# csm-kr/faster_rcnn_pytorch

Hardware: AMD Instinct MI355X
Metric: train images/sec (VGG16 Faster R-CNN, 600x1000, bs=1/GPU) (higher is better)
Workload: dtype f32; 1 GPU; VGG16 Faster R-CNN train step, synthetic 600x1000 frames, bs=1/GPU, HIP proposal/RoI path (N=20646 anchors, pre/post NMS 12000/2000, 128 RoIs, RoIPool 7x7 on 512x37x62); global_batch=1, parallelism=dp1, submission=eager (one launch per kernel), sampling=device-philox

## Files before the change

### faster_rcnn_pytorch_amd/csrc/rpn_conv_f32.hip

```cpp
#include "frcnn_common.h"
#include "frcnn_internal.h"
#include "frcnn_layout.h"
#include <algorithm>
#include <atomic>
#include <cstdlib>
#include <cstring>
#include <type_traits>
FRCNN_LAYOUT_STAMP(rpn_conv_f32);

typedef float f32x16 __attribute__((ext_vector_type(16)));

#define CF_MT 128
#define CF_NT 128
#define CF_CI 4
#define CF_KK (CF_CI * 9)
#define CF_AS 37
#define CF_RS 144
#define CF_ROWS (CF_CI * 3)
#define CF_SLAB (CF_MT * CF_NT)
#define CF_MAX_TILES 32768

struct CfLevel { const float *x; float *y; int H, W, HW, tile0; };
struct CfArgs {
    CfLevel lv[FRCNN_MAX_LEVELS];
    int n_levels, C, n_co_tiles, n_pos_tiles, Kc, n_units, G, pos_major;
};
struct CfTile { const float *x; float *y; int W, HW, p0, co0, tile; };

__device__ __forceinline__ CfTile cf_tile(const CfArgs &a, int t)
{
    int ct, pt;
    if (a.pos_major) { pt = t / a.n_co_tiles; ct = t - pt * a.n_co_tiles; }
    else { ct = t / a.n_pos_tiles; pt = t - ct * a.n_pos_tiles; }
    int l = 0;
#pragma unroll
    for (int q = 1; q < FRCNN_MAX_LEVELS; ++q) l += (q < a.n_levels && pt >= a.lv[q].tile0) ? 1 : 0;
    CfTile T;
    T.x = a.lv[l].x; T.y = a.lv[l].y; T.W = a.lv[l].W; T.HW = a.lv[l].HW;
    T.p0 = (pt - a.lv[l].tile0) * CF_NT;
    T.co0 = ct * CF_MT;
    T.tile = t;
    return T;
}

__device__ __forceinline__ long long cf_start(int s, int U, int G) { return ((long long)s * U) / G; }

#ifndef CF_WPS
#define CF_WPS 2
#endif
__global__ __launch_bounds__(256, CF_WPS) void rpn_conv3x3_f32_kernel(CfArgs a, const float *__restrict__ w, float *__restrict__ part, int *__restrict__ cnt)
{
    __shared__ float sA[2][CF_MT * CF_AS];
    __shared__ float sB[2][CF_ROWS * CF_RS];
    __shared__ int s_last;
    const int tid = threadIdx.x, lane = tid & 63, wave = __builtin_amdgcn_readfirstlane(tid >> 6);
    const int wm = wave >> 1, wn = wave & 1, li = lane & 31, lh = lane >> 5;
    const int G = a.G, U = a.n_units, Kc = a.Kc;
    const int sigma = (G % 8 == 0) ? (int)(blockIdx.x & 7) * (G >> 3) + (int)(blockIdx.x >> 3) : (int)blockIdx.x;
    const int u0 = (int)cf_start(sigma, U, G), u1 = (int)cf_start(sigma + 1, U, G);
    if (u0 >= u1) return;
    const int Ktot = a.C * 9;

    unsigned a_off[5];
    int a_lds[5];
#pragma unroll
    for (int q = 0; q < 5; ++q) {
        const int idx = tid + 256 * q, row = idx / 9, pc = idx - row * 9;
        a_off[q] = (unsigned)(row * Ktot + pc * 4);
        a_lds[q] = row * CF_AS + pc * 4;
    }
    const int hi = tid >> 7, bj = tid & 127;
    const int h_row = (tid >> 1) % CF_ROWS, h_ci = h_row / 3, h_dy = h_row - 3 * h_ci - 1, h_j = (tid & 1) ? CF_NT : -1;
    const bool a_tail = tid < 128, b_tail = tid < 2 * CF_ROWS;
    float4 ra[5];
    float rb[7];
    unsigned rb_ok = 0;
    auto issue_loads = [&](const CfTile &T, int chunk) {
        const float *wb = w + (size_t)T.co0 * Ktot + chunk * CF_KK;
        const float *xb = T.x + (size_t)chunk * CF_CI * T.HW;
#pragma unroll
        for (int q = 0; q < 5; ++q)
            if (q < 4 || a_tail) ra[q] = *(const float4 *)(wb + a_off[q]);
        unsigned okm = 0;
#pragma unroll
        for (int q = 0; q < 7; ++q) {
            int ci, dy, j;
            if (q < 6) { ci = hi ? (2 * q + 1) / 3 : (2 * q) / 3; dy = hi ? (2 * q + 1) % 3 - 1 : (2 * q) % 3 - 1; j = bj; }
            else { ci = h_ci; dy = h_dy; j = h_j; }
            const int f = T.p0 + j + dy * T.W;
            const bool ok = f >= 0 && f < T.HW && (q < 6 || b_tail);
// ... 480 lines not shown
#pragma unroll
                for (int i = 0; i < 3; ++i)
#pragma unroll
                    for (int j = 0; j < 3; ++j) w9[i][j] = wc[(i - 1) * (wt + 2) + (j - 1)];
#pragma unroll
                for (int r = 0; r < IN; ++r)
#pragma unroll
                    for (int q = 0; q < IN; ++q) {
                        const int tr = r == 0 ? 0 : (r <= M ? 1 : 2), br = r == 0 ? M - 1 : (r <= M ? r - 1 : 0);
                        const int tc = q == 0 ? 0 : (q <= M ? 1 : 2), bc = q == 0 ? M - 1 : (q <= M ? q - 1 : 0);
                        d[r][q] = ((w9[tr][tc] >> (br * M + bc)) & 1u) ? d[r][q] : 0.0f;
                    }
            }
        }
        if (MODE == 1) {
#pragma unroll
            for (int r = 0; r < IN; ++r)
#pragma unroll
                for (int q = 0; q < IN; ++q) bsum += d[r][q];
        }
        float wv[A][IN];
#pragma unroll
        for (int q = 0; q < IN; ++q) {
            float col[IN], o[A];
#pragma unroll
            for (int r = 0; r < IN; ++r) col[r] = d[r][q];
            if (MODE != 1) wn_bt<M>(col, o); else wn_a<M>(col, o);
#pragma unroll
            for (int r = 0; r < A; ++r) wv[r][q] = o[r];
        }
        const size_t at = col0 + (size_t)(ty0 + rr) * tw + tx0 + txl;
#pragma unroll
        for (int r = 0; r < A; ++r) {
            float o[A];
            if (MODE != 1) wn_bt<M>(wv[r], o); else wn_a<M>(wv[r], o);
#pragma unroll
#if defined(WN_TABL) && (WN_TABL & 2)
            for (int q = 0; q < A; ++q) if (o[q] == 1.2345e-30f) V[(size_t)(r * A + q) * plane + at] = o[q];
#else
            for (int q = 0; q < A; ++q) V[(size_t)(r * A + q) * plane + at] = o[q];
#endif
        }
        if (MODE == 2) {
            float w2[A][M];
#pragma unroll
            for (int r = 0; r < M; ++r)
#pragma unroll
                for (int q = 0; q < M; ++q) bsum += d[r + 1][q + 1];
#pragma unroll
            for (int q = 0; q < M; ++q) {
                float col[M], o[A];
#pragma unroll
                for (int r = 0; r < M; ++r) col[r] = d[r + 1][q + 1];
                wn_a<M>(col, o);
#pragma unroll
                for (int r = 0; r < A; ++r) w2[r][q] = o[r];
            }
#pragma unroll
            for (int r = 0; r < A; ++r) {
                float o[A];
                wn_a<M>(w2[r], o);
#pragma unroll
                for (int q = 0; q < A; ++q) a.out2[(size_t)(r * A + q) * plane + at] = o[q];
            }
        }
    }
    if (MODE != 0 && a.db_part) {
        __shared__ float red[4];
#pragma unroll
        for (int h = 32; h > 0; h >>= 1) bsum += __shfl_down(bsum, h, 64);
        if ((threadIdx.x & 63) == 0) red[threadIdx.x >> 6] = bsum;
        __syncthreads();
        if (threadIdx.x == 0) a.db_part[(size_t)c * st.first[FRCNN_MAX_LEVELS] + blockIdx.x] = (red[0] + red[1]) + (red[2] + red[3]);
    }
    if (a.zero_pad && strip == 0) {
        const int T = a.lv[l].T, Tp = (T + a.tg - 1) / a.tg * a.tg, np = Tp - T;
        for (int e = threadIdx.x; e < P * np; e += 256) {
            const int xi = e / np, q = e - xi * np;
            (MODE == 2 ? a.out2 : V)[(size_t)xi * plane + col0 + T + q] = 0.0f;
        }
    }
}

template <int M, bool POOL>
__device__ __forceinline__ void wn_output_tile(const WnArgs &a, int c, int t, const float (&mv)[Wn<M>::P])
{
    constexpr int A = Wn<M>::A;
    int l = 0;
#pragma unroll
    for (int q = 1; q < FRCNN_MAX_LEVELS; ++q) l += (q < a.n_levels && t >= a.lv[q].off) ? 1 : 0;
    const int tl = t - a.lv[l].off;
    if (tl >= a.lv[l].T) return;
    const size_t at = (size_t)c * a.Ttot + t;
    float s[M][A];
#pragma unroll
    for (int q = 0; q < A; ++q) {
        float col[A], o[M];
#pragma unroll
        for (int r = 0; r < A; ++r) col[r] = mv[r * A + q];
        wn_at<M>(col, o);
#pragma unroll
        for (int i = 0; i < M; ++i) s[i][q] = o[i];
    }
    const float b = a.bias ? a.bias[c] : 0.0f;
    const int H = a.lv[l].H, W = a.lv[l].W, ty = tl / a.lv[l].tw, tx = tl - ty * a.lv[l].tw;
    unsigned word = 0;
    if (POOL) {
        float v[M][M];
#pragma unroll
        for (int i = 0; i < M; ++i) {
            float o[M];
            wn_at<M>(s[i], o);
#pragma unroll
            for (int j = 0; j < M; ++j) { const float t = o[j] + b; v[i][j] = t < 0.0f ? 0.0f : t; }
        }
        const int Hp = H >> 1, Wp = W >> 1;
        float *yp = a.lv[l].y + (size_t)c * Hp * Wp;
#pragma unroll
        for (int wi = 0; wi < 2; ++wi)
#pragma unroll
            for (int wj = 0; wj < 2; ++wj) {
                const int py = 2 * ty + wi, px = 2 * tx + wj;
                if (py < Hp && px < Wp) {
                    float mx = v[2 * wi][2 * wj];
                    unsigned arg = 0;
                    if (v[2 * wi][2 * wj + 1] > mx || v[2 * wi][2 * wj + 1] != v[2 * wi][2 * wj + 1]) { mx = v[2 * wi][2 * wj + 1]; arg = 1; }
                    if (v[2 * wi + 1][2 * wj] > mx || v[2 * wi + 1][2 * wj] != v[2 * wi + 1][2 * wj]) { mx = v[2 * wi + 1][2 * wj]; arg = 2; }
                    if (v[2 * wi + 1][2 * wj + 1] > mx || v[2 * wi + 1][2 * wj + 1] != v[2 * wi + 1][2 * wj + 1]) { mx = v[2 * wi + 1][2 * wj + 1]; arg = 3; }
                    yp[(size_t)py * Wp + px] = mx;
                    word |= (arg | (mx > 0.0f ? 4u : 0u)) << (3 * (wi * 2 + wj));
                }
            }
        if (a.bits_out) a.bits_out[at] = (unsigned short)word;
        return;
    }
    float *y = a.lv[l].y + (size_t)c * H * W + (size_t)(M * ty) * W + M * tx;
    const bool vec = (W % M) == 0 && ((size_t)a.lv[l].y & (4 * M - 1)) == 0, pairs = (W & 1) == 0 && ((size_t)a.lv[l].y & 7) == 0;
#pragma unroll
    for (int i = 0; i < M; ++i) {
        float o[M];
        wn_at<M>(s[i], o);
        if (M * ty + i < H) {
            float v[M];
#pragma unroll
            for (int j = 0; j < M; ++j) {
                v[j] = o[j] + b;
                if (a.relu) v[j] = v[j] < 0.0f ? 0.0f : v[j];
                if (M * tx + j < W) word |= (v[j] > 0.0f) ? (1u << (i * M + j)) : 0u;
            }
            if (vec) {
                if (M == 4) *(float4 *)(y + (size_t)i * W) = make_float4(v[0], v[1], v[2], v[3]);
                else *(float2 *)(y + (size_t)i * W) = make_float2(v[0], v[1]);
            } else if (M == 4 && pairs) {
#pragma unroll
                for (int j = 0; j < M; j += 2)
                    if (M * tx + j < W) *(float2 *)(y + (size_t)i * W + j) = make_float2(v[j], v[j + 1]);
            } else {
#pragma unroll
                for (int j = 0; j < M; ++j)
                    if (M * tx + j < W) y[(size_t)i * W + j] = v[j];
            }
        }
    }
    if (a.bits_out) a.bits_out[at] = (unsigned short)word;
}

template <int M, bool POOL>
__global__ __launch_bounds__(256) void rpn_wino_output_kernel(WnArgs a, const float *__restrict__ Mp)
{
    static_assert(!POOL || M == 4, "fused pooling: 4 x 4 tiles only");
    constexpr int A = Wn<M>::A, P = Wn<M>::P;
    const int t = blockIdx.x * 256 + threadIdx.x, c = blockIdx.y;
    if (t >= a.Ttot) return;
    const size_t plane = (size_t)a.C * a.Ttot, at = (size_t)c * a.Ttot + t;
    float mv[P];
#pragma unroll
    for (int q = 0; q < A; ++q)
#pragma unroll
        for (int r = 0; r < A; ++r) {
#if defined(WN_TABL) && (WN_TABL & 4)
            mv[r * A + q] = (float)(r + q); asm volatile("" : "+v"(mv[r * A + q]));
#else
            mv[r * A + q] = Mp[(size_t)(r * A + q) * plane + at];
#endif
        }
    wn_output_tile<M, POOL>(a, c, t, mv);
}

template <int M>
__global__ __launch_bounds__(256) void rpn_wino_dw_kernel(const float *__restrict__ dU, float *__restrict__ dw, unsigned n, float *__restrict__ db,
                                                          const float *__restrict__ db_part, int n_strips)
{
    constexpr int A = Wn<M>::A;
    const unsigned dw_blocks = (n + 255u) / 256u;
    if (blockIdx.x >= dw_blocks) {
        __shared__ float red[256];
        const unsigned c = blockIdx.x - dw_blocks;
        float t = 0.0f;
        for (int i = threadIdx.x; i < n_strips; i += 256) t += db_part[(size_t)c * n_strips + i];
        red[threadIdx.x] = t;
        __syncthreads();
#pragma unroll
        for (int h = 128; h > 0; h >>= 1) {
            if ((int)threadIdx.x < h) red[threadIdx.x] += red[threadIdx.x + h];
            __syncthreads();
        }
        if (threadIdx.x == 0) db[c] = red[0];
        return;
    }
    const unsigned o = blockIdx.x * 256u + threadIdx.x;
    if (o >= n) return;
    float t[3][A];
#pragma unroll
    for (int q = 0; q < A; ++q) {
        float col[A], w3[3];
#pragma unroll
        for (int r = 0; r < A; ++r) col[r] = dU[(size_t)(r * A + q) * n + o];
        wn_gt<M>(col, w3);
#pragma unroll
        for (int i = 0; i < 3; ++i) t[i][q] = w3[i];
    }
#pragma unroll
    for (int i = 0; i < 3; ++i) {
        float w3[3];
        wn_gt<M>(t[i], w3);
#pragma unroll
        for (int j = 0; j < 3; ++j) dw[(size_t)o * 9 + i * 3 + j] = w3[j];
    }
}

#ifdef WN_STAMP
__device__ unsigned long long wn_stamps[4 * 1024];
extern "C" __attribute__((visibility("default"))) int frcnn_debug_wn_stamps(unsigned long long *out)
{
    return (int)hipMemcpyFromSymbol(out, HIP_SYMBOL(wn_stamps), sizeof(wn_stamps));
}
#define WN_STAMP_AT(i) do { if (threadIdx.x == 0) wn_stamps[blockIdx.x * 4 + (i)] = wall_clock64(); } while (0)
#else
#define WN_STAMP_AT(i) do { } while (0)
#endif
typedef short wn_bf16x8 __attribute__((ext_vector_type(8)));
typedef unsigned wn_u32x4 __attribute__((ext_vector_type(4)));
__device__ __forceinline__ void wn_cut8(const float *v, wn_u32x4 &h, wn_u32x4 &m, wn_u32x4 &l)
{
#pragma unroll
    for (int p = 0; p < 4; ++p) {
        const unsigned x0 = __builtin_bit_cast(unsigned, v[2 * p]), x1 = __builtin_bit_cast(unsigned, v[2 * p + 1]);
// ... 242 lines not shown
            const int fsw = (li >> 1) & 7;
            f32x4 fa[2][MI], fb[2][NI];
            auto fetch4 = [&](int j, int slot) {
                const int o = (((4 * lh + j) ^ fsw) << 2);
#pragma unroll
                for (int mi = 0; mi < MI; ++mi) fa[slot][mi] = *(const f32x4 *)(ra + mi * 32 * WN_KC + o);
#pragma unroll
                for (int ni = 0; ni < NI; ++ni) fb[slot][ni] = *(const f32x4 *)(rb + ni * 32 * WN_KC + o);
            };
            fetch4(0, 0);
#pragma unroll
            for (int j = 0; j < 4; ++j) {
                const int slot = j & 1;
                if (j + 1 < 4) fetch4(j + 1, slot ^ 1);
#pragma unroll
                for (int e = 0; e < 4; ++e) {
                    __builtin_amdgcn_sched_barrier(0);
#pragma unroll
                    for (int mi = 0; mi < MI; ++mi)
#pragma unroll
                        for (int ni = 0; ni < NI; ++ni)
                            acc[mi][ni] = __builtin_amdgcn_mfma_f32_32x32x2f32(fa[slot][mi][e], fb[slot][ni][e], acc[mi][ni], 0, 0, 0);
                    __builtin_amdgcn_sched_barrier(0);
                    WN_PIECE(4 * j + e);
                }
                __builtin_amdgcn_sched_barrier(0);
            }
        } else {
            const float *pa = &sA[buf][lh * MT + wm * (MT / 2) + MI * li];
            const float *pb = &sB[buf][lh * NW + wn * (NW / 2) + NI * li];
            float oa[2][MI], ob[2][NI];
            auto fetch = [&](int s, int slot) {
#if defined(WN_ABL) && (WN_ABL & 4)
#pragma unroll
                for (int mi = 0; mi < MI; ++mi) { oa[slot][mi] = (float)s; asm volatile("" : "+v"(oa[slot][mi])); }
#pragma unroll
                for (int ni = 0; ni < NI; ++ni) { ob[slot][ni] = (float)s; asm volatile("" : "+v"(ob[slot][ni])); }
                return;
#endif
                if constexpr (MI == 2) { const float2 t = *(const float2 *)(pa + 2 * s * MT); oa[slot][0] = t.x; oa[slot][1] = t.y; }
                else oa[slot][0] = pa[2 * s * MT];
                if constexpr (NI == 2) { const float2 t = *(const float2 *)(pb + 2 * s * NW); ob[slot][0] = t.x; ob[slot][1] = t.y; }
                else ob[slot][0] = pb[2 * s * NW];
            };
            fetch(0, 0);
#pragma unroll
            for (int s = 0; s < 16; ++s) {
                const int slot = s & 1;
                if (s + 1 < 16) fetch(s + 1, slot ^ 1);
                __builtin_amdgcn_sched_barrier(0);
#pragma unroll
                for (int mi = 0; mi < MI; ++mi)
#pragma unroll
                    for (int ni = 0; ni < NI; ++ni)
                        acc[mi][ni] = __builtin_amdgcn_mfma_f32_32x32x2f32(oa[slot][mi], ob[slot][ni], acc[mi][ni], 0, 0, 0);
                __builtin_amdgcn_sched_barrier(0);
                WN_PIECE(s);
            }
        }
#undef WN_PIECE
        if (!more || ntile != tile) {
            if (!more) WN_STAMP_AT(2);
            if constexpr (SPLIT) {
#pragma unroll
                for (int mi = 0; mi < MI; ++mi)
#pragma unroll
                    for (int ni = 0; ni < NI; ++ni) acc[mi][ni] += accs[mi][ni];
            }
            finish_segment(T, seg_first, chunk + 1 - seg_first);
            if (!more) WN_STAMP_AT(3);
            zero_acc();
            seg_first = 0;
            if (more) T = Tn;
        }
        tile = ntile; chunk = nchunk;
        asm volatile("s_waitcnt vmcnt(0)" ::: "memory");
#if !(defined(WN_ABL) && (WN_ABL & 8))
        __syncthreads();
#endif
    }
}

typedef float wn_f32x4 __attribute__((ext_vector_type(4)));
#define WO_TB 32
#define WO_NB 4
__device__ __forceinline__ void wn_dma16(const float *g, const float *lds)
{
    const unsigned l = (unsigned)(size_t)(const __attribute__((address_space(3))) float *)lds;
    asm volatile("s_mov_b32 m0, %0\n\ts_nop 0\n\tglobal_load_lds_dwordx4 %1, off" ::"s"(__builtin_amdgcn_readfirstlane(l)), "v"(g) : "memory");
}
template <int K, bool POOL>
__global__ __launch_bounds__(256, 1) void rpn_wino_gemm_out64_kernel(WnArgs a, const float *__restrict__ U, const float *__restrict__ V)
{
    constexpr int P = 36, MO = 64, NS = K / 4, bufF = K * (MO + WO_TB), NB = WO_NB;
    constexpr int TPW = K / 16 + K / 32;
    extern __shared__ __attribute__((aligned(16))) float wo_s[];
    const int tid = threadIdx.x, lane = tid & 63, wave = __builtin_amdgcn_readfirstlane(tid >> 6), i16 = lane & 15, kk = lane >> 4;
    const int t0 = blockIdx.x * WO_TB;
    const size_t sU = (size_t)K * MO, sV = (size_t)K * a.Ttot;
    auto issue = [&](int xi, int buf) {
        float *sA = wo_s + buf * bufF, *sB = sA + K * MO;
        const float *u = U + (size_t)xi * sU, *v = V + (size_t)xi * sV + t0;
#pragma unroll
        for (int q = 0; q < K / 16; ++q) {
            const int d = wave + 4 * q, r = lane >> 4, c = ((lane & 15) * 4 - 16 * r) & 63;
            wn_dma16(u + (size_t)(4 * d + r) * MO + c, sA + d * 256);
        }
#pragma unroll
        for (int q = 0; q < K / 32; ++q) {
            const int d = wave + 4 * q, r = lane >> 3, c = ((lane & 7) * 4 - 16 * ((r & 3) >> 1)) & 31;
            wn_dma16(v + (size_t)(8 * d + r) * a.Ttot + c, sB + d * 256);
        }
    };
    wn_f32x4 acc[P][2];
#pragma unroll
    for (int xi = 0; xi < P; ++xi) { acc[xi][0] = (wn_f32x4){0.0f, 0.0f, 0.0f, 0.0f}; acc[xi][1] = (wn_f32x4){0.0f, 0.0f, 0.0f, 0.0f}; }
#pragma unroll
    for (int xi = 0; xi < NB - 1; ++xi) issue(xi, xi);
#pragma unroll
    for (int xi = 0; xi < P; ++xi) {
        {
            const int fl = (P - 1 - xi) < (NB - 2) ? (P - 1 - xi) : (NB - 2);
            static_assert(NB - 2 <= 2, "counted waits below");
            if (fl == 2) asm volatile("s_waitcnt vmcnt(%0)" ::"n"(2 * TPW) : "memory");
            else if (fl == 1) asm volatile("s_waitcnt vmcnt(%0)" ::"n"(TPW) : "memory");
            else asm volatile("s_waitcnt vmcnt(0)" ::: "memory");
        }
        __syncthreads();
#if !(defined(WO_ABL) && (WO_ABL & 1))
        if (xi + NB - 1 < P) issue(xi + NB - 1, (xi + NB - 1) % NB);
#endif
        const float *sA = wo_s + (xi % NB) * bufF, *sB = sA + K * MO;
        const float *pa = sA + kk * MO + ((wave * 16 + i16 + 16 * kk) & 63);
        const float *pb0 = sB + kk * WO_TB + ((i16 + 16 * (kk >> 1)) & 31), *pb1 = sB + kk * WO_TB + ((16 + i16 + 16 * (kk >> 1)) & 31);
#pragma unroll
        for (int s = 0; s < NS; ++s) {
            const float av = pa[s * 4 * MO], b0 = pb0[s * 4 * WO_TB], b1 = pb1[s * 4 * WO_TB];
#if defined(WO_ABL) && (WO_ABL & 2)
            if (s > 0) continue;
#endif
            acc[xi][0] = __builtin_amdgcn_mfma_f32_16x16x4f32(av, b0, acc[xi][0], 0, 0, 0);
            acc[xi][1] = __builtin_amdgcn_mfma_f32_16x16x4f32(av, b1, acc[xi][1], 0, 0, 0);
        }
    }
#pragma unroll
    for (int tb = 0; tb < 2; ++tb)
#pragma unroll
        for (int r = 0; r < 4; ++r) {
            float mv[P];
#pragma unroll
            for (int xi = 0; xi < P; ++xi) mv[xi] = acc[xi][tb][r];
            wn_output_tile<4, POOL>(a, wave * 16 + 4 * kk + r, t0 + 16 * tb + i16, mv);
        }
}

static std::atomic<int> g_wn_products{[] { const char *e = getenv("FRCNN_CONV_F32_PRODUCTS"); return (e && (!strcmp(e, "split") || !strcmp(e, "1"))) ? 1 : 0; }()};
FRCNN_EXPORT int frcnn_conv3x3_f32_products(int mode)
{
    if (mode < 0) return g_wn_products.load();
    return g_wn_products.exchange(mode ? 1 : 0);
}

static int wn_launch_gemm(bool nt, int MT, int NW, const WgArgs &g, float *part, int *cnt, hipStream_t s)
{
    const bool split = g_wn_products.load() != 0;
#define WN_GEMM_CASE(NTv, MTv, NWv)                                                                                          \
    if (nt == NTv && MT == MTv && NW == NWv) {                                                                               \
        if (split) FRCNN_LAUNCH((rpn_wino_gemm_kernel<NTv, MTv, NWv, true>), dim3((unsigned)g.G), dim3(256), 0, s, g, part, cnt);   \
        else FRCNN_LAUNCH((rpn_wino_gemm_kernel<NTv, MTv, NWv, false>), dim3((unsigned)g.G), dim3(256), 0, s, g, part, cnt); \
        FRCNN_CHECK_LAUNCH("rpn_wino_gemm_kernel");                                                                          \
        return FRCNN_OK;                                                                                                     \
    }
    WN_GEMM_CASE(false, 128, 128)
    WN_GEMM_CASE(false, 64, 128)
    WN_GEMM_CASE(false, 128, 64)
    WN_GEMM_CASE(false, 64, 64)
    WN_GEMM_CASE(true, 128, 128)
    WN_GEMM_CASE(true, 128, 64)
    WN_GEMM_CASE(true, 64, 128)
    WN_GEMM_CASE(true, 64, 64)
#undef WN_GEMM_CASE
    return frcnn_set_error(FRCNN_ERR_UNSUPPORTED, "conv3x3_f32: no GEMM for a %d x %d tile", MT, NW);
}

#define CW_TC 16
#define CW_YS 17
#define CW_XS 19
#define CW_YB (32 * CW_YS)
#define CW_XB (32 * CW_XS)
#define CW_WAVE_LDS (2 * CW_YB + 4 * CW_XB)

struct CwLevel { const float *x; const float *dy; int H, W, HW, n_strips, unit0; };
struct CwArgs {
    CwLevel lv[FRCNN_MAX_LEVELS];
    int n_levels, C, n_units, S;
};

#ifndef CW_WPS
#define CW_WPS 1
#endif
__global__ __launch_bounds__(256, CW_WPS) void rpn_conv3x3_f32_wgrad_kernel(CwArgs a, float *__restrict__ dw, float *__restrict__ part, int *__restrict__ cnt)
{
    __shared__ float s_all[4 * CW_WAVE_LDS];
    __shared__ int s_last;
    const int tid = threadIdx.x, lane = tid & 63, wave = __builtin_amdgcn_readfirstlane(tid >> 6);
    const int li = lane & 31, lh = lane >> 5;
    const int C = a.C, nt = C / 32;
    const int tile = (int)blockIdx.x / a.S, split = (int)blockIdx.x - tile * a.S;
    const int co0 = (tile / nt) * 32, ci0 = (tile % nt) * 32;
    float *sY = s_all + wave * CW_WAVE_LDS, *sX = sY + 2 * CW_YB;
    const int q = split * 4 + wave, nq = a.S * 4;
    const int u0 = (int)(((long long)q * a.n_units) / nq), u1 = (int)(((long long)(q + 1) * a.n_units) / nq);

    f32x16 acc[9];
#pragma unroll
    for (int t = 0; t < 9; ++t)
#pragma unroll
        for (int r = 0; r < 16; ++r) acc[t][r] = 0.0f;

    const int sr = lane >> 1, sh = lane & 1;
    float *wy = sY + sr * CW_YS + sh * 8;
    float *wx = sX + sr * CW_XS + sh * 9;
    unsigned yo[8], xo[9];
    unsigned ymask = 0, xmask = 0;
    int lvl = 0, strip = 0, row = 0, H = 1, W = 1;
    const float *xg = nullptr, *yg = nullptr;
    auto decode = [&](int u) {
        int l = 0;
#pragma unroll
        for (int k = 1; k < FRCNN_MAX_LEVELS; ++k) l += (k < a.n_levels && u >= a.lv[k].unit0) ? 1 : 0;
        const int v = u - a.lv[l].unit0;
        lvl = l; H = a.lv[l].H; W = a.lv[l].W; xg = a.lv[l].x; yg = a.lv[l].dy;
        strip = v / H; row = v - strip * H;
        const int HW = a.lv[l].HW, c0 = strip * CW_TC;
        ymask = 0; xmask = 0;
#pragma unroll
// ... 257 lines not shown
}
FRCNN_EXPORT size_t frcnn_rpn_conv3x3_f32_workspace(const int *H_host, const int *W_host, int n_levels, int C)
{
    if (C <= 0 || C % CF_MT != 0) return 0;
    return frcnn_conv3x3_f32_workspace(H_host, W_host, n_levels, C, C);
}

template <int M>
static int wn_strips(WnStrips *st, const WnArgs &a, const int *H, int n_levels, long long channels, int halo, size_t *lds_bytes, int sm = M)
{
    int n_strips = 0;
    for (int per_block = Wn<M>::TPB; per_block >= 256; per_block /= 2) {
        n_strips = 0;
        for (int l = 0; l < FRCNN_MAX_LEVELS; ++l) {
            st->first[l] = n_strips;
            const int tw = l < n_levels ? a.lv[l].tw : 1, th = l < n_levels ? (H[l] + M - 1) / M : 1;
            st->segs[l] = (tw + Wn<M>::WT - 1) / Wn<M>::WT;
            st->rows[l] = std::min(128, std::max(1, per_block / std::min(tw, Wn<M>::WT)));
            if (l < n_levels) n_strips += st->segs[l] * ((th + st->rows[l] - 1) / st->rows[l]);
        }
        st->first[FRCNN_MAX_LEVELS] = n_strips;
        if ((long long)n_strips * channels >= 4096) break;
    }
    size_t fl = 0;
    for (int l = 0; l < n_levels; ++l) {
        const int wt = std::min(a.lv[l].tw, Wn<M>::WT), th = (H[l] + M - 1) / M, nr = std::min(st->rows[l], th);
        fl = std::max(fl, (size_t)(sm * nr + 2 * halo) * (size_t)(sm * wt + 2 * halo));
    }
    *lds_bytes = fl * sizeof(float);
    return n_strips;
}

template <int M>
static int wn_run(const float *const *in, float *const *out, const unsigned short *bits_in, const int *H, const int *W, int n_levels, int Cin, int Cout,
                  const float *w, bool transposed, const float *bias, int relu, unsigned short *bits_out, float *xt, void *workspace, hipStream_t s,
                  bool pooled = false, const float *u_rot = nullptr, float *dm_out = nullptr, bool want_bias = false)
{
    constexpr int P = Wn<M>::P;
    const int K = transposed ? Cout : Cin, Mo = transposed ? Cin : Cout;
    WnArgs a;
    const long long Ttot = wn_fill(&a, M, in, out, H, W, n_levels);
    a.bits = bits_in;
    FRCNN_REQUIRE(Ttot < (1ll << 24) && (long long)P * std::max(K, Mo) * Ttot < (1ll << 31) * 4, "conv3x3_f32: %lld output tiles are too many", Ttot);
    const CfWs ws = wn_carve(workspace, Cin, Cout, M, Ttot);
    const int MT = Mo % CF_MT == 0 ? CF_MT : 64;
    const int n_m_tiles = Mo / MT, n_t_tiles = (int)(Ttot / a.tg), Kc = K / WN_KC;
    const long long n_tiles = (long long)P * n_m_tiles * n_t_tiles, units = n_tiles * Kc;
    FRCNN_REQUIRE(n_tiles <= CF_MAX_TILES && units < (1ll << 31), "conv3x3_f32: %lld tiles above the limit %d", n_tiles, CF_MAX_TILES);
    const unsigned wb = (unsigned)((Mo / 16) * (K / 16));
    const float *Uuse = ws.U;
    if (transposed && u_rot) Uuse = u_rot;
    else {
        FRCNN_LAUNCH(rpn_wino_weight_kernel<M>, dim3(!transposed && u_rot ? 2 * wb : wb), dim3(256), 0, s, w, ws.U, (float *)u_rot, Cout, Cin, transposed ? 1 : 0);
        FRCNN_CHECK_LAUNCH("rpn_wino_weight_kernel");
    }
    a.C = K;
    float *Vb = xt ? xt : ws.V;
    a.zero_pad = xt ? 1 : 0;
    WnStrips st;
    size_t lds = 0;
    FRCNN_REQUIRE(!pooled || M == 4, "conv3x3_f32: a pooled gradient on the %d x %d tile", M, M);
    const int n_strips = wn_strips<M>(&st, a, H, n_levels, K, 1, &lds, pooled ? 2 : M);
    if (dm_out) {
        a.out2 = dm_out; a.zero_pad = 1;
        if (want_bias) {
            const size_t C9 = (size_t)((std::max(Cin, Cout) + CF_MT - 1) / CF_MT) * CF_MT;
            FRCNN_REQUIRE((size_t)K * n_strips <= C9 * C9 * 9, "conv3x3_f32_bwd_data: %d strips are too many for the bias partials", n_strips);
            a.db_part = ws.wt;
        }
        if (pooled) {
            if constexpr (M == 4) FRCNN_LAUNCH((rpn_wino_input_kernel<4, 2, true>), dim3((unsigned)n_strips, (unsigned)K), dim3(256), lds, s, a, st, Vb);
        } else FRCNN_LAUNCH((rpn_wino_input_kernel<M, 2, false>), dim3((unsigned)n_strips, (unsigned)K), dim3(256), lds, s, a, st, Vb);
    } else if (pooled) {
        if constexpr (M == 4) FRCNN_LAUNCH((rpn_wino_input_kernel<4, 0, true>), dim3((unsigned)n_strips, (unsigned)K), dim3(256), lds, s, a, st, Vb);
    } else FRCNN_LAUNCH((rpn_wino_input_kernel<M, 0, false>), dim3((unsigned)n_strips, (unsigned)K), dim3(256), lds, s, a, st, Vb);
    FRCNN_CHECK_LAUNCH("rpn_wino_input_kernel");
    if constexpr (M == 4) {
        static const bool no_fuse = [] { const char *e = getenv("FRCNN_WINO_NO_FUSE"); return e && atoi(e) != 0; }();
        if (Mo == 64 && K == 64 && !no_fuse) {
            a.C = Mo; a.bias = bias; a.relu = relu; a.bits_out = bits_out;
            const size_t wl = (size_t)WO_NB * K * (64 + WO_TB) * sizeof(float);
            if (relu == 2) (void)hipFuncSetAttribute((const void *)rpn_wino_gemm_out64_kernel<64, true>, hipFuncAttributeMaxDynamicSharedMemorySize, (int)wl);
            else (void)hipFuncSetAttribute((const void *)rpn_wino_gemm_out64_kernel<64, false>, hipFuncAttributeMaxDynamicSharedMemorySize, (int)wl);
            const dim3 gr((unsigned)(Ttot / WO_TB));
            if (relu == 2) FRCNN_LAUNCH((rpn_wino_gemm_out64_kernel<64, true>), gr, dim3(256), wl, s, a, Uuse, Vb);
            else FRCNN_LAUNCH((rpn_wino_gemm_out64_kernel<64, false>), gr, dim3(256), wl, s, a, Uuse, Vb);
            FRCNN_CHECK_LAUNCH("rpn_wino_gemm_out64_kernel");
            return FRCNN_OK;
        }
    }
    WgArgs g = {Uuse, Vb, ws.M, (long long)Mo * K, (long long)K * Ttot, (long long)Mo * Ttot, Mo, (int)Ttot, (int)Ttot,
                n_m_tiles, n_t_tiles, Kc, (int)units, (int)std::min<long long>(cf_ranges(), units), 0};
    {
        const long long per = (n_tiles + g.G - 1) / g.G;
        if (n_tiles >= 2ll * g.G && per * g.G * 100 <= n_tiles * 116) g.whole = 1;
        else if (n_tiles <= g.G && n_tiles * WN_ONE_TILE_DEN >= (long long)g.G * WN_ONE_TILE_NUM) { g.G = (int)n_tiles; g.whole = 1; }
    }
    { const int rc = wn_launch_gemm(false, MT, a.tg, g, ws.part, ws.cnt, s); if (rc) return rc; }
    a.C = Mo; a.bias = bias; a.relu = relu; a.bits_out = bits_out;
    if (relu == 2) {
        if constexpr (M == 4) FRCNN_LAUNCH((rpn_wino_output_kernel<4, true>), dim3((unsigned)((Ttot + 255) / 256), (unsigned)Mo), dim3(256), 0, s, a, ws.M);
    } else FRCNN_LAUNCH((rpn_wino_output_kernel<M, false>), dim3((unsigned)((Ttot + 255) / 256), (unsigned)Mo), dim3(256), 0, s, a, ws.M);
    FRCNN_CHECK_LAUNCH("rpn_wino_output_kernel");
    return FRCNN_OK;
}

static int cf_check(const void *const *p0, const void *const *p1, const int *H, const int *W, int n_levels, int Cin, int Cout, int in_mult, int out_mult,
                    const void *w, void *ws, size_t ws_bytes, const char *what)
{
    FRCNN_REQUIRE(p0 && p1 && H && W && w && ws, "%s: NULL pointer", what);
    FRCNN_REQUIRE(n_levels >= 1 && n_levels <= FRCNN_MAX_LEVELS, "%s: 1 <= n_levels <= %d", what, FRCNN_MAX_LEVELS);
    if (!wn_dims_ok(Cin, Cout) || Cin % in_mult != 0 || Cout % out_mult != 0)
        return frcnn_set_error(FRCNN_ERR_UNSUPPORTED, "%s: Cin=%d / Cout=%d must be multiples of %d / %d", what, Cin, Cout, in_mult, out_mult);
    for (int l = 0; l < n_levels; ++l) {
        FRCNN_REQUIRE(p0[l] && p1[l] && H[l] > 0 && W[l] > 0, "%s: bad level %d", what, l);
        FRCNN_REQUIRE((long long)H[l] * W[l] * std::max(Cin, Cout) < (1ll << 31), "%s: level %d too large", what, l);
    }
    const size_t need = frcnn_conv3x3_f32_workspace(H, W, n_levels, Cin, Cout);
    if (ws_bytes < need) return frcnn_set_error(FRCNN_ERR_WORKSPACE, "%s: workspace %zu < %zu bytes", what, ws_bytes, need);
    return FRCNN_OK;
}

FRCNN_EXPORT int frcnn_conv3x3_f32_fwd(const float *const *x_dev, float *const *y_dev, const int *H_host, const int *W_host, int n_levels, int Cin, int Cout,
                                       const float *w_dev, const float *bias_dev, int relu, unsigned short *relu_bits_dev, float *x_transformed_dev, float *u_rotated_dev,
                                       void *workspace, size_t workspace_bytes, void *stream)
{
    int rc = cf_check((const void *const *)x_dev, (const void *const *)y_dev, H_host, W_host, n_levels, Cin, Cout, WN_KC, 64, w_dev, workspace, workspace_bytes,
                      "conv3x3_f32_fwd");
    if (rc) return rc;
    FRCNN_REQUIRE(relu >= 0 && relu <= 2, "conv3x3_f32_fwd: relu = %d (0 none, 1 ReLU, 2 ReLU + max_pool2d(2, 2))", relu);
    if (relu == 2 && wn_pick_m(H_host, W_host, n_levels) != 4)
        return frcnn_set_error(FRCNN_ERR_UNSUPPORTED, "conv3x3_f32_fwd: the fused max-pool needs the 4 x 4 tile (frcnn_conv3x3_f32_tile_size)");
    if (wn_pick_m(H_host, W_host, n_levels) == 4)
        return wn_run<4>(x_dev, y_dev, nullptr, H_host, W_host, n_levels, Cin, Cout, w_dev, false, bias_dev, relu, relu_bits_dev, x_transformed_dev, workspace, (hipStream_t)stream,
                         false, u_rotated_dev);
    return wn_run<2>(x_dev, y_dev, nullptr, H_host, W_host, n_levels, Cin, Cout, w_dev, false, bias_dev, relu, relu_bits_dev, x_transformed_dev, workspace, (hipStream_t)stream,
                     false, u_rotated_dev);
}

FRCNN_EXPORT int frcnn_conv3x3_f32_supported(const int *H_host, const int *W_host, int n_levels, int Cin, int Cout, int need_grads)
{
    if (!H_host || !W_host || n_levels < 1 || n_levels > FRCNN_MAX_LEVELS || !wn_dims_ok(Cin, Cout) || Cout % 64 != 0 || (need_grads && Cin % 64 != 0)) return 0;
    const int M = wn_pick_m(H_host, W_host, n_levels), P = (M + 2) * (M + 2), Cm = std::max(Cin, Cout);
    WnArgs a;
    const long long Ttot = wn_fill(&a, M, nullptr, nullptr, H_host, W_host, n_levels);
    for (int l = 0; l < n_levels; ++l)
        if (H_host[l] <= 0 || W_host[l] <= 0 || (long long)H_host[l] * W_host[l] * Cm >= (1ll << 31)) return 0;
    if (Ttot >= (1ll << 24) || (long long)P * Cm * Ttot >= (1ll << 31) * 4) return 0;
    auto side = [](long long c) { return c % CF_MT == 0 ? c / CF_MT : c / 64; };
    auto tiles_ok = [&](long long mt, long long nt, long long k_chunks) {
        const long long n = P * mt * nt;
        return n <= CF_MAX_TILES && n * k_chunks < (1ll << 31);
    };
    if (!tiles_ok(side(Cout), Ttot / a.tg, Cin / WN_KC)) return 0;
    if (need_grads && (!tiles_ok(side(Cin), Ttot / a.tg, Cout / WN_KC) || !tiles_ok(side(Cout), side(Cin), Ttot / WN_KC))) return 0;
    return 1;
}

FRCNN_EXPORT int frcnn_conv3x3_f32_tile_size(const int *H_host, const int *W_host, int n_levels)
{
    if (!H_host || !W_host || n_levels < 1 || n_levels > FRCNN_MAX_LEVELS) return 0;
    return wn_pick_m(H_host, W_host, n_levels);
}

FRCNN_EXPORT size_t frcnn_conv3x3_f32_relu_bits_words(const int *H_host, const int *W_host, int n_levels, int Cout)
{
    if (!H_host || !W_host || n_levels < 1 || n_levels > FRCNN_MAX_LEVELS || Cout <= 0) return 0;
    WnArgs a;
    return (size_t)Cout * (size_t)wn_fill(&a, wn_pick_m(H_host, W_host, n_levels), nullptr, nullptr, H_host, W_host, n_levels);
// ... 172 lines not shown
```

Measured before the change: 154.0 images/s.

## Make fused Winograd GEMM+output kernel persistent with 512 threads and streaming inverse transform

Reworks the fused 64-channel Winograd GEMM/output kernel into a persistent kernel. Each block covers a contiguous range of 16-tile groups in passes of 64 tiles and uses 8 waves. The DMA ring carries on across passes, and addresses are passed as SGPR bases. Planes are consumed in column order so the inverse transform accumulates row by row, replacing 36 live accumulators per tile with 6 partial accumulators plus a 4x4 output. The aim is to cut register pressure, raise per-block tile width and overlap loads across passes; the cost is a more intricate counted-wait schedule and a grid sized to the CU count.

```diff
diff --git a/faster_rcnn_pytorch_amd/csrc/rpn_conv_f32.hip b/faster_rcnn_pytorch_amd/csrc/rpn_conv_f32.hip
--- a/faster_rcnn_pytorch_amd/csrc/rpn_conv_f32.hip
+++ b/faster_rcnn_pytorch_amd/csrc/rpn_conv_f32.hip
@@ -6,6 +6,7 @@
 #include <cstdlib>
 #include <cstring>
 #include <type_traits>
+#include <utility>
 FRCNN_LAYOUT_STAMP(rpn_conv_f32);
 
 typedef float f32x16 __attribute__((ext_vector_type(16)));
@@ -652,38 +653,26 @@
     }
 }
 
+__device__ __forceinline__ bool wn_tile_level(const WnArgs &a, int t, int &l, int &tl)
+{
+    l = 0;
+#pragma unroll
+    for (int q = 1; q < FRCNN_MAX_LEVELS; ++q) l += (q < a.n_levels && t >= a.lv[q].off) ? 1 : 0;
+    tl = t - a.lv[l].off;
+    return tl < a.lv[l].T;
+}
 template <int M, bool POOL>
-__device__ __forceinline__ void wn_output_tile(const WnArgs &a, int c, int t, const float (&mv)[Wn<M>::P])
-{
-    constexpr int A = Wn<M>::A;
-    int l = 0;
-#pragma unroll
-    for (int q = 1; q < FRCNN_MAX_LEVELS; ++q) l += (q < a.n_levels && t >= a.lv[q].off) ? 1 : 0;
-    const int tl = t - a.lv[l].off;
-    if (tl >= a.lv[l].T) return;
+__device__ __forceinline__ void wn_output_finish(const WnArgs &a, int l, int tl, int c, int t, float b, const float (&o)[M][M])
+{
     const size_t at = (size_t)c * a.Ttot + t;
-    float s[M][A];
-#pragma unroll
-    for (int q = 0; q < A; ++q) {
-        float col[A], o[M];
-#pragma unroll
-        for (int r = 0; r < A; ++r) col[r] = mv[r * A + q];
-        wn_at<M>(col, o);
-#pragma unroll
-        for (int i = 0; i < M; ++i) s[i][q] = o[i];
-    }
-    const float b = a.bias ? a.bias[c] : 0.0f;
     const int H = a.lv[l].H, W = a.lv[l].W, ty = tl / a.lv[l].tw, tx = tl - ty * a.lv[l].tw;
     unsigned word = 0;
     if (POOL) {
         float v[M][M];
 #pragma unroll
-        for (int i = 0; i < M; ++i) {
-            float o[M];
-            wn_at<M>(s[i], o);
-#pragma unroll
-            for (int j = 0; j < M; ++j) { const float t = o[j] + b; v[i][j] = t < 0.0f ? 0.0f : t; }
-        }
+        for (int i = 0; i < M; ++i)
+#pragma unroll
+            for (int j = 0; j < M; ++j) { const float t = o[i][j] + b; v[i][j] = t < 0.0f ? 0.0f : t; }
         const int Hp = H >> 1, Wp = W >> 1;
         float *yp = a.lv[l].y + (size_t)c * Hp * Wp;
 #pragma unroll
@@ -708,13 +697,11 @@
     const bool vec = (W % M) == 0 && ((size_t)a.lv[l].y & (4 * M - 1)) == 0, pairs = (W & 1) == 0 && ((size_t)a.lv[l].y & 7) == 0;
 #pragma unroll
     for (int i = 0; i < M; ++i) {
-        float o[M];
-        wn_at<M>(s[i], o);
         if (M * ty + i < H) {
             float v[M];
 #pragma unroll
             for (int j = 0; j < M; ++j) {
-                v[j] = o[j] + b;
+                v[j] = o[i][j] + b;
                 if (a.relu) v[j] = v[j] < 0.0f ? 0.0f : v[j];
                 if (M * tx + j < W) word |= (v[j] > 0.0f) ? (1u << (i * M + j)) : 0u;
             }
@@ -733,6 +720,28 @@
         }
     }
     if (a.bits_out) a.bits_out[at] = (unsigned short)word;
+}
+template <int M, bool POOL>
+__device__ __forceinline__ void wn_output_tile(const WnArgs &a, int c, int t, const float (&mv)[Wn<M>::P])
+{
+    constexpr int A = Wn<M>::A;
+    int l, tl;
+    if (!wn_tile_level(a, t, l, tl)) return;
+    float s[M][A];
+#pragma unroll
+    for (int q = 0; q < A; ++q) {
+        float col[A], o[M];
+#pragma unroll
+        for (int r = 0; r < A; ++r) col[r] = mv[r * A + q];
+        wn_at<M>(col, o);
+#pragma unroll
+        for (int i = 0; i < M; ++i) s[i][q] = o[i];
+    }
+    const float b = a.bias ? a.bias[c] : 0.0f;
+    float o[M][M];
+#pragma unroll
+    for (int i = 0; i < M; ++i) wn_at<M>(s[i], o[i]);
+    wn_output_finish<M, POOL>(a, l, tl, c, t, b, o);
 }
 
 template <int M, bool POOL>
@@ -1141,76 +1150,157 @@
 }
 
 typedef float wn_f32x4 __attribute__((ext_vector_type(4)));
-#define WO_TB 32
+#define WO_TB 64
 #define WO_NB 4
+#define WO_TPW 4
 __device__ __forceinline__ void wn_dma16(const float *g, const float *lds)
 {
     const unsigned l = (unsigned)(size_t)(const __attribute__((address_space(3))) float *)lds;
     asm volatile("s_mov_b32 m0, %0\n\ts_nop 0\n\tglobal_load_lds_dwordx4 %1, off" ::"s"(__builtin_amdgcn_readfirstlane(l)), "v"(g) : "memory");
 }
+__device__ __forceinline__ void wn_dma16s(const float *g, unsigned off_bytes, unsigned lds_bytes)
+{
+    asm volatile("s_mov_b32 m0, %0\n\ts_nop 0\n\tglobal_load_lds_dwordx4 %1, %2" ::"s"(__builtin_amdgcn_readfirstlane(lds_bytes)), "v"(off_bytes), "s"(g) : "memory");
+}
+template <class F, int... J> __device__ __forceinline__ void wo_planes(F &&f, std::integer_sequence<int, J...>) { (f(std::integral_constant<int, J>{}), ...); }
 template <int K, bool POOL>
-__global__ __launch_bounds__(256, 1) void rpn_wino_gemm_out64_kernel(WnArgs a, const float *__restrict__ U, const float *__restrict__ V)
-{
-    constexpr int P = 36, MO = 64, NS = K / 4, bufF = K * (MO + WO_TB), NB = WO_NB;
-    constexpr int TPW = K / 16 + K / 32;
+__global__ __launch_bounds__(512, 1) void rpn_wino_gemm_out64_kernel(WnArgs a, const float *__restrict__ U, const float *__restrict__ V)
+{
+    static_assert(K == 64, "the transfer split below is for K = 64");
+    constexpr int P = 36, MO = 64, NS = K / 4, bufF = K * (MO + WO_TB), NB = WO_NB, TPW = WO_TPW;
+    static_assert(P % NB == 0, "the ring runs on across passes: plane xi always sits in buffer xi % NB");
+    static_assert(TPW == (K / 4 + K / 4) / 8 && NB == 4, "counted waits below");
     extern __shared__ __attribute__((aligned(16))) float wo_s[];
     const int tid = threadIdx.x, lane = tid & 63, wave = __builtin_amdgcn_readfirstlane(tid >> 6), i16 = lane & 15, kk = lane >> 4;
-    const int t0 = blockIdx.x * WO_TB;
+    const int wc = wave & 3, half = wave >> 2;
     const size_t sU = (size_t)K * MO, sV = (size_t)K * a.Ttot;
-    auto issue = [&](int xi, int buf) {
-        float *sA = wo_s + buf * bufF, *sB = sA + K * MO;
-        const float *u = U + (size_t)xi * sU, *v = V + (size_t)xi * sV + t0;
-#pragma unroll
-        for (int q = 0; q < K / 16; ++q) {
-            const int d = wave + 4 * q, r = lane >> 4, c = ((lane & 15) * 4 - 16 * r) & 63;
-            wn_dma16(u + (size_t)(4 * d + r) * MO + c, sA + d * 256);
-        }
-#pragma unroll
-        for (int q = 0; q < K / 32; ++q) {
-            const int d = wave + 4 * q, r = lane >> 3, c = ((lane & 7) * 4 - 16 * ((r & 3) >> 1)) & 31;
-            wn_dma16(v + (size_t)(8 * d + r) * a.Ttot + c, sB + d * 256);
+    const int ng = a.Ttot >> 4;
+    const int g0 = (int)(((long long)blockIdx.x * ng) / gridDim.x), g1 = (int)(((long long)(blockIdx.x + 1) * ng) / gridDim.x);
+    const int tend = g1 * 16;
+    auto pass_len = [&](int t) { const int rem = tend - t; return rem >= 64 ? 64 : rem >= 32 ? 32 : rem; };
+    const int lr = lane >> 4, lc = ((lane & 15) * 4 - 16 * lr) & 63;
+    const unsigned offU = (unsigned)(lr * MO + lc) * 4u, offV = (unsigned)((size_t)lr * a.Ttot + lc) * 4u;
+    const unsigned lds0 = __builtin_amdgcn_readfirstlane((unsigned)(size_t)(const __attribute__((address_space(3))) float *)wo_s + (unsigned)wave * 1024u);
+    auto issue = [&](int j, int tb0, int len) {
+        const int xi = (j % 6) * 6 + j / 6, buf = j % NB;
+        const unsigned lA = lds0 + (unsigned)(buf * bufF) * 4u, lB = lA + K * MO * 4u;
+        const float *ub = U, *vb = V;
+        size_t sv = sV;
+        asm volatile("" : "+s"(ub), "+s"(vb), "+s"(sv));
+        const float *u = ub + (size_t)xi * sU, *v = vb + (size_t)xi * sv + tb0;
+#pragma unroll
+        for (int q = 0; q < 2; ++q) {
+            const int d = wave + 8 * q;
+            wn_dma16s(u + (size_t)(4 * d) * MO, offU, lA + q * 8192u);
+        }
+#pragma unroll
+        for (int q = 0; q < 2; ++q) {
+            const int d = wave + 8 * q;
+            const float *src = v + (size_t)(4 * d) * a.Ttot;
+            if (lc < len) wn_dma16s(src, offV, lB + q * 8192u);
         }
     };
-    wn_f32x4 acc[P][2];
-#pragma unroll
-    for (int xi = 0; xi < P; ++xi) { acc[xi][0] = (wn_f32x4){0.0f, 0.0f, 0.0f, 0.0f}; acc[xi][1] = (wn_f32x4){0.0f, 0.0f, 0.0f, 0.0f}; }
-#pragma unroll
-    for (int xi = 0; xi < NB - 1; ++xi) issue(xi, xi);
-#pragma unroll
-    for (int xi = 0; xi < P; ++xi) {
-        {
-            const int fl = (P - 1 - xi) < (NB - 2) ? (P - 1 - xi) : (NB - 2);
-            static_assert(NB - 2 <= 2, "counted waits below");
-            if (fl == 2) asm volatile("s_waitcnt vmcnt(%0)" ::"n"(2 * TPW) : "memory");
-            else if (fl == 1) asm volatile("s_waitcnt vmcnt(%0)" ::"n"(TPW) : "memory");
+    float bias[4];
+#pragma unroll
+    for (int r = 0; r < 4; ++r) bias[r] = a.bias ? a.bias[wc * 16 + 4 * kk + r] : 0.0f;
+    int t0 = g0 * 16, len = pass_len(t0);
+    if (t0 < tend) {
+#pragma unroll
+        for (int j = 0; j < NB - 1; ++j) issue(j, t0, len);
+    }
+    while (t0 < tend) {
+        const int tn = t0 + len, nlen = pass_len(tn);
+        const bool more = tn < tend;
+        const bool act0 = 32 * half < len, act1 = 32 * half + 16 < len;
+        wn_f32x4 acc[6][2], Y[4][4][2];
+#pragma unroll
+        for (int i = 0; i < 4; ++i)
+#pragma unroll
+            for (int bq = 0; bq < 4; ++bq) { Y[i][bq][0] = (wn_f32x4){0.0f, 0.0f, 0.0f, 0.0f}; Y[i][bq][1] = (wn_f32x4){0.0f, 0.0f, 0.0f, 0.0f}; }
+        auto plane = [&](auto jc) {
+            constexpr int j = decltype(jc)::value, q = j / 6, r = j % 6;
+            if (j == 0) asm volatile("s_waitcnt vmcnt(0)" ::: "memory");
+            else if (j < P - 2) asm volatile("s_waitcnt vmcnt(%0)" ::"n"(2 * TPW) : "memory");
+            else if (more) asm volatile("s_waitcnt vmcnt(%0)" ::"n"(2 * TPW) : "memory");
             else asm volatile("s_waitcnt vmcnt(0)" ::: "memory");
-        }
-        __syncthreads();
+            __syncthreads();
 #if !(defined(WO_ABL) && (WO_ABL & 1))
-        if (xi + NB - 1 < P) issue(xi + NB - 1, (xi + NB - 1) % NB);
+            if (j + NB - 1 < P) issue(j + NB - 1, t0, len);
+            else if (more) issue(j + NB - 1 - P, tn, nlen);
 #endif
-        const float *sA = wo_s + (xi % NB) * bufF, *sB = sA + K * MO;
-        const float *pa = sA + kk * MO + ((wave * 16 + i16 + 16 * kk) & 63);
-        const float *pb0 = sB + kk * WO_TB + ((i16 + 16 * (kk >> 1)) & 31), *pb1 = sB + kk * WO_TB + ((16 + i16 + 16 * (kk >> 1)) & 31);
-#pragma unroll
-        for (int s = 0; s < NS; ++s) {
-            const float av = pa[s * 4 * MO], b0 = pb0[s * 4 * WO_TB], b1 = pb1[s * 4 * WO_TB];
+            if (r == 0) { acc[0][0] = acc[0][1] = acc[1][0] = acc[1][1] = acc[2][0] = acc[2][1] = acc[3][0] = acc[3][1] = acc[4][0] = acc[4][1] = acc[5][0] = acc[5][1] = (wn_f32x4){0.0f, 0.0f, 0.0f, 0.0f}; }
+            const float *sA = wo_s + (j % NB) * bufF, *sB = sA + K * MO;
+            const float *pa = sA + kk * MO + ((wc * 16 + i16 + 16 * kk) & 63);
+            const float *pb0 = sB + kk * WO_TB + ((32 * half + i16 + 16 * kk) & 63), *pb1 = sB + kk * WO_TB + ((32 * half + 16 + i16 + 16 * kk) & 63);
+#pragma unroll
+            for (int s = 0; s < NS; ++s) {
 #if defined(WO_ABL) && (WO_ABL & 2)
-            if (s > 0) continue;
+                if (s > 0) continue;
 #endif
-            acc[xi][0] = __builtin_amdgcn_mfma_f32_16x16x4f32(av, b0, acc[xi][0], 0, 0, 0);
-            acc[xi][1] = __builtin_amdgcn_mfma_f32_16x16x4f32(av, b1, acc[xi][1], 0, 0, 0);
-        }
-    }
-#pragma unroll
-    for (int tb = 0; tb < 2; ++tb)
-#pragma unroll
-        for (int r = 0; r < 4; ++r) {
-            float mv[P];
-#pragma unroll
-            for (int xi = 0; xi < P; ++xi) mv[xi] = acc[xi][tb][r];
-            wn_output_tile<4, POOL>(a, wave * 16 + 4 * kk + r, t0 + 16 * tb + i16, mv);
-        }
+                const float av = pa[s * 4 * MO], b0 = pb0[s * 4 * WO_TB], b1 = pb1[s * 4 * WO_TB];
+                acc[r][0] = __builtin_amdgcn_mfma_f32_16x16x4f32(av, b0, acc[r][0], 0, 0, 0);
+                acc[r][1] = __builtin_amdgcn_mfma_f32_16x16x4f32(av, b1, acc[r][1], 0, 0, 0);
+            }
+#if !(defined(WO_ABL) && (WO_ABL & 4))
+            if (r == 5) {
+#pragma unroll
+                for (int tb = 0; tb < 2; ++tb)
+#pragma unroll
+                    for (int e = 0; e < 4; ++e) {
+                        float col[6], sv[4];
+#pragma unroll
+                        for (int rr = 0; rr < 6; ++rr) col[rr] = acc[rr][tb][e];
+                        wn_at<4>(col, sv);
+#pragma unroll
+                        for (int i = 0; i < 4; ++i) {
+                            const float x = sv[i];
+                            if (q == 0) Y[i][0][tb][e] += x;
+                            else if (q == 1) { Y[i][0][tb][e] += x; Y[i][1][tb][e] += x; Y[i][2][tb][e] += x; Y[i][3][tb][e] += x; }
+                            else if (q == 2) { Y[i][0][tb][e] += x; Y[i][1][tb][e] -= x; Y[i][2][tb][e] += x; Y[i][3][tb][e] -= x; }
+                            else if (q == 3) { Y[i][0][tb][e] += x; Y[i][1][tb][e] = __builtin_fmaf(2.0f, x, Y[i][1][tb][e]); Y[i][2][tb][e] = __builtin_fmaf(4.0f, x, Y[i][2][tb][e]); Y[i][3][tb][e] = __builtin_fmaf(8.0f, x, Y[i][3][tb][e]); }
+                            else if (q == 4) { Y[i][0][tb][e] += x; Y[i][1][tb][e] = __builtin_fmaf(-2.0f, x, Y[i][1][tb][e]); Y[i][2][tb][e] = __builtin_fmaf(4.0f, x, Y[i][2][tb][e]); Y[i][3][tb][e] = __builtin_fmaf(-8.0f, x, Y[i][3][tb][e]); }
+                            else Y[i][3][tb][e] += x;
+                        }
+                    }
+#pragma unroll
+                for (int tb = 0; tb < 2; ++tb)
+                    asm volatile("" : "+v"(Y[0][0][tb]), "+v"(Y[0][1][tb]), "+v"(Y[0][2][tb]), "+v"(Y[0][3][tb]), "+v"(Y[1][0][tb]), "+v"(Y[1][1][tb]), "+v"(Y[1][2][tb]),
+                                 "+v"(Y[1][3][tb]), "+v"(Y[2][0][tb]), "+v"(Y[2][1][tb]), "+v"(Y[2][2][tb]), "+v"(Y[2][3][tb]), "+v"(Y[3][0][tb]), "+v"(Y[3][1][tb]),
+                                 "+v"(Y[3][2][tb]), "+v"(Y[3][3][tb]));
+            }
+#else
+            if (r == 5) {
+#pragma unroll
+                for (int tb = 0; tb < 2; ++tb)
+#pragma unroll
+                    for (int rr = 0; rr < 6; ++rr) Y[rr & 3][q & 3][tb] += acc[rr][tb];
+            }
+#endif
+        };
+        wo_planes(plane, std::make_integer_sequence<int, P>{});
+        auto kp = __builtin_amdgcn_kernarg_segment_ptr();
+        asm volatile("" : "+s"(kp));
+        const WnArgs &a = *(const WnArgs *)kp;
+#pragma unroll
+        for (int tb = 0; tb < 2; ++tb) {
+            if (!(tb ? act1 : act0)) continue;
+            const int t = t0 + 32 * half + 16 * tb + i16;
+            int l, tl;
+            if (!wn_tile_level(a, t, l, tl)) continue;
+#pragma unroll
+            for (int e = 0; e < 4; ++e) {
+                float o[4][4];
+#pragma unroll
+                for (int i = 0; i < 4; ++i)
+#pragma unroll
+                    for (int bq = 0; bq < 4; ++bq) o[i][bq] = Y[i][bq][tb][e];
+                int c = wc * 16 + 4 * kk + e;
+                asm volatile("" : "+v"(c));
+                wn_output_finish<4, POOL>(a, l, tl, c, t, bias[e], o);
+            }
+        }
+        t0 = tn; len = nlen;
+    }
 }
 
 static std::atomic<int> g_wn_products{[] { const char *e = getenv("FRCNN_CONV_F32_PRODUCTS"); return (e && (!strcmp(e, "split") || !strcmp(e, "1"))) ? 1 : 0; }()};
@@ -1634,9 +1724,9 @@
             const size_t wl = (size_t)WO_NB * K * (64 + WO_TB) * sizeof(float);
             if (relu == 2) (void)hipFuncSetAttribute((const void *)rpn_wino_gemm_out64_kernel<64, true>, hipFuncAttributeMaxDynamicSharedMemorySize, (int)wl);
             else (void)hipFuncSetAttribute((const void *)rpn_wino_gemm_out64_kernel<64, false>, hipFuncAttributeMaxDynamicSharedMemorySize, (int)wl);
-            const dim3 gr((unsigned)(Ttot / WO_TB));
-            if (relu == 2) FRCNN_LAUNCH((rpn_wino_gemm_out64_kernel<64, true>), gr, dim3(256), wl, s, a, Uuse, Vb);
-            else FRCNN_LAUNCH((rpn_wino_gemm_out64_kernel<64, false>), gr, dim3(256), wl, s, a, Uuse, Vb);
+            const dim3 gr((unsigned)std::min<long long>(cf_ranges() / CF_WPS, Ttot / 16));
+            if (relu == 2) FRCNN_LAUNCH((rpn_wino_gemm_out64_kernel<64, true>), gr, dim3(512), wl, s, a, Uuse, Vb);
+            else FRCNN_LAUNCH((rpn_wino_gemm_out64_kernel<64, false>), gr, dim3(512), wl, s, a, Uuse, Vb);
             FRCNN_CHECK_LAUNCH("rpn_wino_gemm_out64_kernel");
             return FRCNN_OK;
         }
```

After: 155.2 images/s, median of 6. About the same (+0.8%).
